# maxim2266/csvplus

Hardware: AMD Instinct MI355X
Metric: joined rows/sec (IndexOn build + chained Join, 1e8-row 3-col orders) (higher is better)
Workload: dtype u32; 1 GPU; BASELINE configs[3]: orders(1e8 x {cust_id,prod_id,qty}).Join(UniqueIndexOn customers.id 1e7).Join(UniqueIndexOn products.prod_id 1e5); rows=100000000, customers=10000000, products=100000, rows_this_rank=100000000, exchange=none (1 GPU), output=sorted positions

## Files before the change

csvplus_amd/csrc/chain.hip:

```cpp
#include <type_traits>

#include "probe_device.hpp"

namespace cph {

constexpr int kChainThreads = 256;
constexpr int kChainWaves   = kChainThreads / kWave;
constexpr int kChainRows    = 8;
constexpr int kWaveTile     = kWave * kChainRows;
constexpr int kChainTile    = kChainThreads * kChainRows;
constexpr int kChainMasks   = kChainRows * kChainWaves;
constexpr int kMaxChain     = 4;

struct ChainStepArg {
    DevCol col;
    const uint8_t* codec;
    const uint32_t* rowtab;
    const uint2* ranktab;
    int32_t positions;
    int32_t ranktab_lds;
    const uint4* hash;
    uint32_t hash_sectors;
    uint32_t hash_slice_mask;
    int32_t src;
    const uint32_t* src_perm;
    const void* codes;
    const uint32_t* perm;
    uint64_t n_index;
    int32_t codec_bytes;
    int32_t key32;
};
struct ChainArgs {
    ChainStepArg step[kMaxChain];
    uint32_t* out_rows[kMaxChain];
    int32_t nt_streams;
    int32_t reserved_;
};
struct LeanArgs {
    int32_t identity[kMaxChain];
    ArithPlan arith[kMaxChain];
};

template <int S, bool LONG, bool WIDE, bool DBG, uint32_t LEAN = 0, int R = kChainRows, bool DEP = false>
__global__ __launch_bounds__(kChainThreads) void k_chain_dense(ChainArgs a, uint64_t nprobe, uint64_t probe_base,
                                                              uint64_t ntiles, uint64_t* __restrict__ masks,
                                                              uint32_t* __restrict__ wave_counts, int dbg_flags, LeanArgs la) {
    extern __shared__ __attribute__((aligned(16))) uint8_t smem[];
    using B = std::conditional_t<WIDE, uint64_t, uint32_t>;
    using CW = std::conditional_t<WIDE, uint64_t, uint32_t>;
    const int dbg = DBG ? dbg_flags : 0;
    CodecView cv[S];
    {
        uint8_t* p = smem;
#pragma unroll
        for (int s = 0; s < S; s++) {
            if ((LEAN >> s) & 1u) continue;
            cv[s] = codec_load_to_lds(a.step[s].codec, p);
            p += a.step[s].codec_bytes;
        }
    }
    const CPH_LDS uint32_t* rank_lds[S];
    {
        uint8_t* p = smem;
#pragma unroll
        for (int s = 0; s < S; s++) p += a.step[s].codec_bytes;
        bool any = false;
#pragma unroll
        for (int s = 0; s < S; s++) {
            rank_lds[s] = nullptr;
            const int nblk = a.step[s].ranktab_lds;
            if (LEAN != 0 && nblk) {
                uint2* dst = reinterpret_cast<uint2*>(p);
                for (int i = threadIdx.x; i < 2 * nblk; i += kChainThreads) dst[i] = a.step[s].ranktab[i];
                rank_lds[s] = (const CPH_LDS uint32_t*)p;
                p += (size_t)nblk * 16;
                any = true;
            } else if (nblk) {
                uint32_t* dst = reinterpret_cast<uint32_t*>(p);
                for (int i = threadIdx.x; i < nblk; i += kChainThreads) {
                    const uint2 b0 = a.step[s].ranktab[2 * i], b1 = a.step[s].ranktab[2 * i + 1];
                    dst[3 * i] = b0.x;
                    dst[3 * i + 1] = b1.x;
                    dst[3 * i + 2] = b0.x ? b0.y : b1.y;
                }
                rank_lds[s] = (const CPH_LDS uint32_t*)p;
                p += (size_t)((nblk * 12 + 15) & ~15);
                any = true;
            }
        }
        if (any) __syncthreads();
    }
    const int lane = lane_id();
    const uint32_t wave = (uint32_t)__builtin_amdgcn_readfirstlane(wave_id());

#pragma unroll 1
    for (uint64_t tile = blockIdx.x; tile < ntiles; tile += gridDim.x) {
        uint32_t wave_matches = 0;
#pragma unroll 1
      for (int part = 0; part < kChainRows / R; part++) {
        const uint64_t wbase = tile * kChainTile + (uint64_t)wave * kWaveTile + (uint64_t)part * (R * kWave);
        const WaveRows<R> wr = wave_rows<R>(wbase, nprobe);
        uint32_t okm = wr.okm;
        WaveSpans<R, B> sp[S];
        uint64_t c0[S][R], c1[LONG ? S : 1][R];
        CW code[S][R];
        uint32_t brow[S][R];
#pragma unroll
      for (int lvl = 0; lvl < (DEP ? S : 1); lvl++) {
#pragma unroll
        for (int s = 0; s < S; s++) {
            if (DEP && s != lvl) continue;
            if ((LEAN >> s) & 1u) continue;
            if constexpr (DEP) {
                const int32_t src = a.step[s].src;
                if (src != 0) {
                    const int t = (src < 0 ? -src : src) - 1;
                    uint32_t grow[R];
#pragma unroll
                    for (int k = 0; k < R; k++) grow[k] = 0u;
#pragma unroll
                    for (int u = 0; u < S; u++)
                        if (u < s && u == t) {
#pragma unroll
                            for (int k = 0; k < R; k++) grow[k] = (okm >> k) & 1u ? brow[u][k] : 0u;
                        }
                    if (a.step[s].src_perm) {
#pragma unroll
                        for (int k = 0; k < R; k++) grow[k] = a.step[s].src_perm[grow[k]];
                    }
                    gather_spans<R, B>(a.step[s].col, grow, &sp[s]);
                    continue;
                }
            }
            if (a.nt_streams) wave_spans<R, B, false, true>(a.step[s].col, wr, &sp[s]);
            else wave_spans<R, B>(a.step[s].col, wr, &sp[s]);
        }
#pragma unroll
        for (int s = 0; s < S; s++) {
            if (DEP && s != lvl) continue;
            if ((LEAN >> s) & 1u) {
                typedef const __attribute__((address_space(1))) uint64_t* global_u64_ptr;
                const global_u64_ptr w = (global_u64_ptr)a.step[s].col.data + wr.rbase;
                if (a.nt_streams) {
#pragma unroll
                    for (int k = 0; k < R; k++) c0[s][k] = __builtin_nontemporal_load(&w[wr.rel[k]]);
                } else {
#pragma unroll
                    for (int k = 0; k < R; k++) c0[s][k] = w[wr.rel[k]];
                }
                continue;
            }
#pragma unroll
            for (int k = 0; k < R; k++) {
                c0[s][k] = a.nt_streams ? sp[s].chunk_nt(k, 0) : sp[s].chunk(k, 0);
                if constexpr (LONG) c1[s][k] = a.nt_streams ? sp[s].chunk_nt(k, 1) : sp[s].chunk(k, 1);
            }
        }
#pragma unroll
        for (int s = 0; s < S; s++) {
            if (DEP && s != lvl) continue;
            if (DBG && (dbg & 2)) {
#pragma unroll
                for (int k = 0; k < R; k++) code[s][k] = (CW)((c0[s][k] ^ (LONG ? c1[LONG ? s : 0][k] : 0ull)) & 1023);
            } else if ((LEAN >> s) & 1u) {
                encode_rows_arith<R, CW>(la.arith[s], c0[s], code[s], &okm);
            } else if (!WIDE || cv[s].hdr->lutw_bits == 32) {
                encode_rows<R, uint32_t, B, CW, LONG>(cv[s], sp[s], c0[s], c1[LONG ? s : 0], code[s], &okm,
                                                               a.step[s].col.fixed_width != 0 && (int)a.step[s].col.fixed_width == cv[s].hdr->col_maxlen[0]);
            } else {
                encode_rows<R, uint64_t, B, CW, LONG>(cv[s], sp[s], c0[s], c1[LONG ? s : 0], code[s], &okm,
                                                               a.step[s].col.fixed_width != 0 && (int)a.step[s].col.fixed_width == cv[s].hdr->col_maxlen[0]);
            }
        }
#pragma unroll
        for (int s = 0; s < S; s++) {
            if (DEP && s != lvl) continue;
            const ChainStepArg& st = a.step[s];
            if constexpr (LEAN != 0) {
                if (la.identity[s]) {
#pragma unroll
                    for (int k = 0; k < R; k++)
                        brow[s][k] = ((okm >> k) & 1u) && (uint32_t)code[s][k] < (uint32_t)st.n_index ? (uint32_t)code[s][k] : kTableAbsent;
                } else if (rank_lds[s]) {
#pragma unroll
                    for (int k = 0; k < R; k++) {
                        const uint32_t cidx = (okm >> k) & 1u ? (uint32_t)code[s][k] : 0u;
                        const CPH_LDS uint32_t* e = rank_lds[s] + 2u * (cidx >> 5);
                        const uint32_t bits = e[0], before = e[1], bit = cidx & 31u;
                        brow[s][k] = (bits >> bit) & 1u ? before + (uint32_t)__popc(bits & ((1u << bit) - 1u)) : kTableAbsent;
                    }
                } else {
                    uint2 blk[R];
#pragma unroll
                    for (int k = 0; k < R; k++) {
                        const uint32_t cidx = (okm >> k) & 1u ? (uint32_t)code[s][k] : 0u;
                        blk[k] = st.ranktab[cidx >> 5];
                    }
#pragma unroll
                    for (int k = 0; k < R; k++) {
                        const uint32_t bit = (uint32_t)code[s][k] & 31u;
                        brow[s][k] = (blk[k].x >> bit) & 1u ? blk[k].y + (uint32_t)__popc(blk[k].x & ((1u << bit) - 1u)) : kTableAbsent;
                    }
                }
            } else if (st.ranktab) {
                if (rank_lds[s]) {
#pragma unroll
                    for (int k = 0; k < R; k++) {
                        const CW cidx = (okm >> k) & 1u ? code[s][k] : (CW)0;
                        const CPH_LDS uint32_t* e = rank_lds[s] + 3u * (uint32_t)((uint64_t)cidx >> 6);
                        const uint32_t bit = (uint32_t)cidx & 63u;
                        const uint64_t bits = (uint64_t)e[0] | ((uint64_t)e[1] << 32);
                        const bool present = (bits >> bit) & 1ull;
                        brow[s][k] = present ? e[2] + (uint32_t)__popcll(bits & ((1ull << bit) - 1ull)) : kTableAbsent;
                    }
                } else {
                    uint2 blk[R];
#pragma unroll
                    for (int k = 0; k < R; k++) {
                        const CW cidx = (okm >> k) & 1u ? code[s][k] : (CW)0;
                        blk[k] = (DBG && (dbg & 1)) ? make_uint2(~0u, 0u) : st.ranktab[(uint64_t)cidx >> 5];
                    }
#pragma unroll
                    for (int k = 0; k < R; k++) {
                        const uint32_t bit = (uint32_t)code[s][k] & 31u;
                        const bool present = (blk[k].x >> bit) & 1u;
                        brow[s][k] = present ? blk[k].y + (uint32_t)__popc(blk[k].x & ((1u << bit) - 1u)) : kTableAbsent;
                    }
                }
            } else if (st.rowtab) {
#pragma unroll
                for (int k = 0; k < R; k++) {
                    const CW cidx = (okm >> k) & 1u ? code[s][k] : (CW)0;
                    brow[s][k] = (DBG && (dbg & 1)) ? 0u : st.rowtab[cidx];
                }
            } else if (st.hash) {
                const HashView hv{st.hash, st.hash_sectors, st.hash_slice_mask};
#pragma unroll
                for (int g = 0; g < R; g += 4) {
                    HashSector sc[4];
                    uint32_t home[4];
#pragma unroll
                    for (int k = 0; k < 4; k++) {
                        home[k] = hash_home(hash_one((uint64_t)code[s][g + k]), hv.nsectors);
                        sc[k] = hash_load_sector(hv, (okm >> (g + k)) & 1u ? home[k] : 0u);
                    }
#pragma unroll
                    for (int k = 0; k < 4; k++) {
                        uint32_t l, a;
                        bool more;
                        bool hit = hash_match16(sc[k], (uint64_t)code[s][g + k], &l, &a, &more);
                        const bool live = (okm >> (g + k)) & 1u;
                        if (live && more) hit = hash_continue16(hv, home[k], (uint64_t)code[s][g + k], &l, &a);
                        brow[s][g + k] = (hit && live && !(DBG && (dbg & 1))) ? (st.positions ? l : a) : kTableAbsent;
                        if (DBG && (dbg & 1)) brow[s][g + k] = 0u;
                    }
                }
            } else {
#pragma unroll
                for (int k = 0; k < R; k++) {
                    brow[s][k] = kTableAbsent;
                    if (!((okm >> k) & 1u)) continue;
                    uint64_t lo;
                    bool hit;
                    if (st.key32) {
                        const uint32_t* cd = reinterpret_cast<const uint32_t*>(st.codes);
                        lo = lower_bound_dev<uint32_t>(cd, 0, st.n_index, (uint32_t)code[s][k]);
                        hit = lo < st.n_index && cd[lo] == (uint32_t)code[s][k];
                    } else {
                        const uint64_t* cd = reinterpret_cast<const uint64_t*>(st.codes);
                        lo = lower_bound_dev<uint64_t>(cd, 0, st.n_index, (uint64_t)code[s][k]);
                        hit = lo < st.n_index && cd[lo] == (uint64_t)code[s][k];
                    }
                    if (hit) brow[s][k] = st.positions ? (uint32_t)lo : st.perm[lo];
                }
            }
        }
#pragma unroll
        for (int s = 0; s < S; s++) {
            if (DEP && s != lvl) continue;
#pragma unroll
            for (int k = 0; k < R; k++)
                if (brow[s][k] == kTableAbsent) okm &= ~(1u << k);
        }
      }
        const uint64_t mword = (tile * kChainWaves + wave) * kChainRows + (uint64_t)part * R;
#pragma unroll
        for (int k = 0; k < R; k++) {
            const bool ok = (okm >> k) & 1u;
            const uint64_t bal = __ballot(ok);
            wave_matches += (uint32_t)__popcll(bal);
            if (lane == 0) masks[mword + k] = bal;
            if (ok && !(DBG && (dbg & 4))) {
#pragma unroll
                for (int s = 0; s < S; s++) {
                    if (a.nt_streams) __builtin_nontemporal_store(brow[s][k], a.out_rows[s] + wr.rbase + wr.rel[k]);
                    else (a.out_rows[s] + wr.rbase)[wr.rel[k]] = brow[s][k];
                }
            }
        }
      }
        if (lane == 0) wave_counts[tile * kChainWaves + wave] = wave_matches;
    }
}

struct CodeStepArg {
    const uint32_t* codes;
    const uint32_t* rowtab;
    const uint2* ranktab;
    uint64_t n_index, table_entries;
    int32_t identity;
    int32_t reserved_;
};
struct CodeArgs {
    CodeStepArg step[kMaxChain];
    uint32_t* out_rows[kMaxChain];
};
template <int S>
__global__ __launch_bounds__(kChainThreads) void k_chain_codes(CodeArgs a, uint64_t nprobe, uint64_t ntiles, uint64_t* __restrict__ masks,
                                                              uint32_t* __restrict__ wave_counts) {
    const int lane = lane_id();
    const uint32_t wave = (uint32_t)__builtin_amdgcn_readfirstlane(wave_id());
#pragma unroll 1
    for (uint64_t tile = blockIdx.x; tile < ntiles; tile += gridDim.x) {
        const uint64_t wbase = tile * kChainTile + (uint64_t)wave * kWaveTile;
        const WaveRows<kChainRows> wr = wave_rows<kChainRows>(wbase, nprobe);
        uint32_t okm = wr.okm;
        uint32_t code[S][kChainRows], brow[S][kChainRows];
#pragma unroll
        for (int s = 0; s < S; s++)
#pragma unroll
            for (int k = 0; k < kChainRows; k++) code[s][k] = (a.step[s].codes + wr.rbase)[wr.rel[k]];
#pragma unroll
        for (int s = 0; s < S; s++) {
            const CodeStepArg& st = a.step[s];
            if (st.identity) {
#pragma unroll
                for (int k = 0; k < kChainRows; k++) brow[s][k] = (uint64_t)code[s][k] < st.n_index ? code[s][k] : kTableAbsent;
            } else if (st.ranktab) {
                uint2 blk[kChainRows];
#pragma unroll
                for (int k = 0; k < kChainRows; k++) {
                    const bool in = (uint64_t)code[s][k] < st.table_entries;
                    blk[k] = st.ranktab[in ? code[s][k] >> 5 : 0u];
                    if (!in) blk[k].x = 0u;
                }
#pragma unroll
                for (int k = 0; k < kChainRows; k++) {
                    const uint32_t bit = code[s][k] & 31u;
                    brow[s][k] = (blk[k].x >> bit) & 1u ? blk[k].y + (uint32_t)__popc(blk[k].x & ((1u << bit) - 1u)) : kTableAbsent;
                }
            } else {
#pragma unroll
                for (int k = 0; k < kChainRows; k++) {
                    const bool in = (uint64_t)code[s][k] < st.table_entries;
                    const uint32_t r = st.rowtab[in ? code[s][k] : 0u];
                    brow[s][k] = in ? r : kTableAbsent;
                }
            }
        }
#pragma unroll
        for (int s = 0; s < S; s++)
#pragma unroll
            for (int k = 0; k < kChainRows; k++)
                if (brow[s][k] == kTableAbsent) okm &= ~(1u << k);
        uint32_t wave_matches = 0;
        const uint64_t mword = (tile * kChainWaves + wave) * kChainRows;
#pragma unroll
        for (int k = 0; k < kChainRows; k++) {
            const bool ok = (okm >> k) & 1u;
            const uint64_t bal = __ballot(ok);
            wave_matches += (uint32_t)__popcll(bal);
            if (lane == 0) masks[mword + k] = bal;
            if (ok) {
#pragma unroll
                for (int s = 0; s < S; s++) (a.out_rows[s] + wr.rbase)[wr.rel[k]] = brow[s][k];
            }
        }
        if (lane == 0) wave_counts[tile * kChainWaves + wave] = wave_matches;
    }
}

__global__ __launch_bounds__(256) void k_sum_counts(const uint32_t* __restrict__ counts, uint64_t n,
                                                   unsigned long long* __restrict__ total) {
    __shared__ uint64_t s_w[256 / kWave];
    uint64_t t = 0;
    const uint64_t stride = (uint64_t)gridDim.x * 256;
    for (uint64_t i = (uint64_t)blockIdx.x * 256 + threadIdx.x; i < n; i += stride) t += counts[i];
    t = wave_sum(t);
    if (lane_id() == 0) s_w[wave_id()] = t;
    __syncthreads();
    if (threadIdx.x == 0) {
        uint64_t r = 0;
        for (int w = 0; w < 256 / kWave; w++) r += s_w[w];
        if (r) atomicAdd(total, (unsigned long long)r);
    }
}

__global__ __launch_bounds__(256) void k_sum_counts_report(const uint32_t* __restrict__ counts, uint64_t n, unsigned long long* __restrict__ acc,
                                                          uint32_t* __restrict__ ticket, unsigned long long* __restrict__ host_out) {
    __shared__ uint64_t s_w[256 / kWave];
    uint64_t t = 0;
    const uint64_t stride = (uint64_t)gridDim.x * 256;
    for (uint64_t i = (uint64_t)blockIdx.x * 256 + threadIdx.x; i < n; i += stride) t += counts[i];
    t = wave_sum(t);
    if (lane_id() == 0) s_w[wave_id()] = t;
    __syncthreads();
    if (threadIdx.x == 0) {
        uint64_t r = 0;
        for (int w = 0; w < 256 / kWave; w++) r += s_w[w];
        if (r) atomicAdd(acc, (unsigned long long)r);
        __threadfence();
        if (atomicAdd(ticket, 1u) == gridDim.x - 1u) {
            const unsigned long long total = atomicExch(acc, 0ull);
            atomicExch(ticket, 0u);
            *host_out = total;
            __threadfence_system();
        }
    }
}

template <int S>
__global__ __launch_bounds__(kChainThreads) void k_chain_compact(ChainArgs dense_rows, uint64_t probe_base,
                                                                const uint64_t* __restrict__ masks,
                                                                const uint32_t* __restrict__ wave_base, uint64_t ntiles,
                                                                uint64_t* __restrict__ out_stream, ChainArgs out_rows) {
    const int lane = lane_id(), wave = wave_id();
    const uint64_t lt = lanemask_lt();
    for (uint64_t tile = blockIdx.x; tile < ntiles; tile += gridDim.x) {
        const uint64_t wt = tile * kChainWaves + wave;
        uint64_t pos = wave_base[wt];
#pragma unroll
        for (int k = 0; k < kChainRows; k++) {
            const uint64_t m = masks[wt * kChainRows + k];
            if ((m >> lane) & 1ull) {
                const uint64_t row = wt * kWaveTile + (uint64_t)k * kWave + lane;
                const uint64_t p = pos + (uint64_t)__popcll(m & lt);
                out_stream[p] = probe_base + row;
#pragma unroll
                for (int s = 0; s < S; s++) out_rows.out_rows[s][p] = dense_rows.out_rows[s][row];
            }
            pos += (uint64_t)__popcll(m);
        }
    }
}

__global__ void k_compose_u64(const uint64_t* __restrict__ src, const uint64_t* __restrict__ idx, uint64_t* __restrict__ dst,
                              uint64_t n) {
    const uint64_t stride = (uint64_t)gridDim.x * blockDim.x;
    for (uint64_t i = (uint64_t)blockIdx.x * blockDim.x + threadIdx.x; i < n; i += stride) dst[i] = src[idx[i]];
}
__global__ void k_compose_u32(const uint32_t* __restrict__ src, const uint64_t* __restrict__ idx, uint32_t* __restrict__ dst,
                              uint64_t n) {
    const uint64_t stride = (uint64_t)gridDim.x * blockDim.x;
    for (uint64_t i = (uint64_t)blockIdx.x * blockDim.x + threadIdx.x; i < n; i += stride) dst[i] = src[idx[i]];
}

__global__ void k_perm_rows(const uint32_t* __restrict__ perm, const uint32_t* __restrict__ pos, uint32_t* __restrict__ dst, uint64_t n) {
    const uint64_t stride = (uint64_t)gridDim.x * blockDim.x;
    for (uint64_t i = (uint64_t)blockIdx.x * blockDim.x + threadIdx.x; i < n; i += stride) dst[i] = perm[pos[i]];
}

__global__ void k_gather_rows(const uint32_t* __restrict__ tab, const uint32_t* __restrict__ idx, uint32_t* __restrict__ dst, uint64_t n) {
    const uint64_t stride = (uint64_t)gridDim.x * blockDim.x;
    for (uint64_t i = (uint64_t)blockIdx.x * blockDim.x + threadIdx.x; i < n; i += stride) dst[i] = tab[idx[i]];
}

struct PrejoinArgs {
    int32_t n;
    int32_t src_dep[kMaxChain - 1];
    const uint32_t* src_rows[kMaxChain - 1];
    const uint32_t* tab[kMaxChain - 1];
    uint32_t* out_rows[kMaxChain - 1];
};
__global__ __launch_bounds__(kChainThreads) void k_chain_prejoined(PrejoinArgs a, uint64_t nprobe, uint64_t ntiles, uint64_t* __restrict__ masks,
                                                                  uint32_t* __restrict__ wave_counts) {
    const int lane = lane_id();
    const uint32_t wave = (uint32_t)__builtin_amdgcn_readfirstlane(wave_id());
#pragma unroll 1
    for (uint64_t tile = blockIdx.x; tile < ntiles; tile += gridDim.x) {
        const uint64_t wbase = tile * kChainTile + (uint64_t)wave * kWaveTile;
        const uint64_t mword = (tile * kChainWaves + wave) * kChainRows;
        uint32_t okm = 0;
#pragma unroll
        for (int k = 0; k < kChainRows; k++) okm |= (uint32_t)((masks[mword + k] >> lane) & 1ull) << k;
        uint32_t val[kMaxChain - 1][kChainRows];
#pragma unroll
        for (int j = 0; j < kMaxChain - 1; j++) {
            if (j >= a.n) break;
            uint32_t h[kChainRows];
            const int sd = a.src_dep[j];
            if (sd < 0) {
#pragma unroll
                for (int k = 0; k < kChainRows; k++) {
                    const uint64_t r = wbase + (uint64_t)k * kWave + lane;
                    h[k] = (okm >> k) & 1u ? a.src_rows[j][r] : 0u;
                }
            } else {
#pragma unroll
                for (int k = 0; k < kChainRows; k++) h[k] = 0u;
#pragma unroll
                for (int u = 0; u < kMaxChain - 1; u++)
                    if (u < j && u == sd) {
#pragma unroll
                        for (int k = 0; k < kChainRows; k++) h[k] = (okm >> k) & 1u ? val[u][k] : 0u;
                    }
            }
#pragma unroll
            for (int k = 0; k < kChainRows; k++) val[j][k] = a.tab[j][h[k]];
#pragma unroll
            for (int k = 0; k < kChainRows; k++)
                if (val[j][k] == kTableAbsent) okm &= ~(1u << k);
        }
        uint32_t wave_matches = 0;
#pragma unroll
        for (int k = 0; k < kChainRows; k++) {
            const bool ok = (okm >> k) & 1u;
            const uint64_t bal = __ballot(ok);
            wave_matches += (uint32_t)__popcll(bal);
            if (lane == 0) masks[mword + k] = bal;
            if (ok) {
                const uint64_t r = wbase + (uint64_t)k * kWave + lane;
#pragma unroll
                for (int j = 0; j < kMaxChain - 1; j++)
                    if (j < a.n) __builtin_nontemporal_store(val[j][k], a.out_rows[j] + r);
            }
        }
        if (lane == 0) wave_counts[tile * kChainWaves + wave] = wave_matches;
    }
}


constexpr int kPjThreads = 256, kPjItems = 8, kPjTile = kPjThreads * kPjItems;
__global__ __launch_bounds__(kPjThreads) void k_prejoin_tuples(const uint32_t* __restrict__ tab, const uint32_t* __restrict__ h,
                                                              const uint32_t* __restrict__ perm, uint64_t n,
                                                              uint32_t* __restrict__ out_v, uint32_t* __restrict__ tile_counts) {
    __shared__ uint32_t s_w[kPjThreads / kWave];
    const uint64_t base = (uint64_t)blockIdx.x * kPjTile;
    uint32_t hv[kPjItems], v[kPjItems];
#pragma unroll
    for (int k = 0; k < kPjItems; k++) {
        const uint64_t i = base + (uint64_t)k * kPjThreads + threadIdx.x;
        hv[k] = i < n ? __builtin_nontemporal_load(h + i) : 0u;
    }
    if (perm) {
#pragma unroll
        for (int k = 0; k < kPjItems; k++) hv[k] = perm[hv[k]];
    }
#pragma unroll
    for (int k = 0; k < kPjItems; k++) v[k] = tab[hv[k]];
    uint32_t cnt = 0;
#pragma unroll
    for (int k = 0; k < kPjItems; k++) {
        const uint64_t i = base + (uint64_t)k * kPjThreads + threadIdx.x;
        if (i < n) {
            __builtin_nontemporal_store(v[k], out_v + i);
            cnt += v[k] != kTableAbsent ? 1u : 0u;
        }
    }
    cnt = wave_sum(cnt);
    if (lane_id() == 0) s_w[wave_id()] = cnt;
    __syncthreads();
    if (threadIdx.x == 0) {
        uint32_t t = 0;
        for (int w = 0; w < kPjThreads / kWave; w++) t += s_w[w];
        tile_counts[blockIdx.x] = t;
    }
}
struct PjCompactArgs {
    int32_t n32;
    const uint32_t* src32[CPH_MAX_CHAIN];
    uint32_t* dst32[CPH_MAX_CHAIN];
    const uint64_t* src64;
    uint64_t* dst64;
};
__global__ __launch_bounds__(kPjThreads) void k_prejoin_compact(PjCompactArgs a, const uint32_t* __restrict__ v, uint64_t n,
                                                               const uint32_t* __restrict__ tile_base) {
    __shared__ uint32_t s_tmp[kPjThreads / kWave + 1];
    const uint64_t i0 = (uint64_t)blockIdx.x * kPjTile + (uint64_t)threadIdx.x * kPjItems;
    uint32_t keep = 0, mine = 0;
#pragma unroll
    for (int k = 0; k < kPjItems; k++)
        if (i0 + k < n && v[i0 + k] != kTableAbsent) {
            keep |= 1u << k;
            mine++;
        }
    uint32_t total;
    uint32_t run = block_exclusive_sum<uint32_t, kPjThreads>(mine, s_tmp, &total);
    uint64_t o = (uint64_t)tile_base[blockIdx.x] + run;
#pragma unroll
    for (int k = 0; k < kPjItems; k++) {
        if (!((keep >> k) & 1u)) continue;
        a.dst64[o] = a.src64[i0 + k];
        for (int j = 0; j < a.n32; j++) a.dst32[j][o] = a.src32[j][i0 + k];
        o++;
    }
}

bool chain_fast_path_ok(const ChainStep* steps, int nsteps) {
    if (nsteps > kMaxChain) return false;
    for (int s = 0; s < nsteps; s++) {
        const cph_index* ix = steps[s].index;
        if (steps[s].ncols != 1 || ix->nkeycols != 1) return false;
        if (ix->first_dup != UINT64_MAX) return false;
        if (ix->codec.nwords != 1 || ix->codec.npos == 0 || !ix->windows.empty()) return false;
// ... 526 lines not shown
```

csvplus_amd/csrc/codec_device.hpp:

```cpp
#pragma once

#include "cph_internal.hpp"
#include "device_utils.hpp"

namespace cph {

__device__ __forceinline__ uint64_t find_first_byte(const uint8_t* data, uint64_t begin, uint64_t len, uint32_t d) {
    const uint64_t dv = 0x0101010101010101ull * (uint64_t)(d & 0xFFu);
    for (uint64_t j = 0; 8 * j < len; j++) {
        const uint64_t x = load_value_chunk(data, begin, len, (int)j) ^ dv;
        const uint64_t t = (x - 0x0101010101010101ull) & ~x & 0x8080808080808080ull;
        if (t) {
            const uint64_t pos = 8 * j + (uint64_t)((__ffsll((long long)t) - 1) >> 3);
            return pos < len ? pos : len;
        }
    }
    return len;
}

__device__ __forceinline__ void value_span_whole(const DevCol& col, uint64_t row, uint64_t* begin, uint64_t* len);
__device__ __forceinline__ void value_span(const DevCol& col, uint64_t row, uint64_t* begin, uint64_t* len) {
    value_span_whole(col, row, begin, len);
    if (col.split) {
        const uint64_t b = *begin, l = *len;
        const uint64_t at = find_first_byte(col.data, b, l, col.split);
        const uint64_t head = at < l ? at + 1 : l;
        if (col.part == 0) {
            *len = head;
        } else {
            *begin = b + head;
            *len = l - head;
        }
    }
}
__device__ __forceinline__ void value_span_whole(const DevCol& col, uint64_t row, uint64_t* begin, uint64_t* len) {
    uint64_t b, l;
    if (col.fixed_width) {
        b = row * (uint64_t)col.fixed_width;
        l = col.fixed_width;
    } else {
        b = load_offset(col.offsets, col.offset_bits, row);
        l = load_offset(col.offsets, col.offset_bits, row + 1) - b;
    }
    const uint64_t s = l < (uint64_t)col.skip ? l : (uint64_t)col.skip;
    b += s;
    l -= s;
    if (col.take != 0xFFFFFFFFu && l > (uint64_t)col.take) l = col.take;
    *begin = b;
    *len = l;
}

#define CPH_LDS __attribute__((address_space(3)))

struct CodecView {
    const CPH_LDS CodecDevHeader* hdr;
    const CPH_LDS uint64_t* mult;
    const CPH_LDS uint8_t* word_of;
    const CPH_LDS uint16_t* lut;
    const CPH_LDS uint8_t* lutw;
    const CPH_LDS uint8_t* unit;
    const CPH_LDS int32_t* dict_off;
    const CPH_LDS int32_t* dict_len;
    const CPH_LDS uint64_t* dict;
    const CPH_LDS int32_t* hash_off;
    const CPH_LDS int32_t* hash_bits;
    const CPH_LDS uint16_t* hash;
    const CPH_LDS WideKey* wide;
    const CPH_LDS uint16_t* wide_hash;
    const CPH_LDS uint16_t* wide_disp;
};

__device__ __forceinline__ CodecView codec_load_to_lds(const uint8_t* g_blob, uint8_t* lds) {
    const CodecDevHeader* gh = reinterpret_cast<const CodecDevHeader*>(g_blob);
    const int total = gh->total_bytes;
    const uint4* src = reinterpret_cast<const uint4*>(g_blob);
    uint4* dst = reinterpret_cast<uint4*>(lds);
    for (int i = threadIdx.x; i < total / 16; i += blockDim.x) dst[i] = src[i];
    __syncthreads();
    const CPH_LDS uint8_t* l = (const CPH_LDS uint8_t*)lds;
    CodecView v;
    v.hdr = (const CPH_LDS CodecDevHeader*)l;
    v.mult = (const CPH_LDS uint64_t*)(l + v.hdr->mult_off);
    v.word_of = l + v.hdr->wordof_off;
    v.lut = (const CPH_LDS uint16_t*)(l + v.hdr->lut_off);
    v.lutw = l + v.hdr->lutw_off;
    v.unit = l + v.hdr->unit_off;
    v.dict_off = (const CPH_LDS int32_t*)(l + v.hdr->dictoff_off);
    v.dict_len = (const CPH_LDS int32_t*)(l + v.hdr->dictlen_off);
    v.dict = (const CPH_LDS uint64_t*)(l + v.hdr->dict_off);
    v.hash_off = (const CPH_LDS int32_t*)(l + v.hdr->hashoff_off);
    v.hash_bits = (const CPH_LDS int32_t*)(l + v.hdr->hashbits_off);
    v.hash = (const CPH_LDS uint16_t*)(l + v.hdr->hash_off);
    v.wide = (const CPH_LDS WideKey*)(l + v.hdr->wide_off);
    v.wide_hash = (const CPH_LDS uint16_t*)(l + v.hdr->wide_hash_off);
    v.wide_disp = (const CPH_LDS uint16_t*)(l + v.hdr->wide_disp_off);
    return v;
}

__device__ __forceinline__ uint32_t wide_slot(const CodecView& cv, uint32_t h) {
    const uint32_t disp = cv.wide_disp[h & ((1u << cv.hdr->wide_disp_bits) - 1u)];
    return ((h >> 16) + disp) & ((1u << cv.hdr->wide_hash_bits) - 1u);
}
__device__ __forceinline__ int wide_lookup(const CodecView& cv, uint64_t w0, uint64_t w1, uint64_t w2, uint64_t w3, uint32_t len) {
    const uint32_t e = cv.wide_hash[wide_slot(cv, wide_hash_lo(w0, w1, w2, w3, len))];
    if (e == 0) return -1;
    const CPH_LDS WideKey* k = cv.wide + (e - 1);
    return k->len == len && k->w[0] == w0 && k->w[1] == w1 && k->w[2] == w2 && k->w[3] == w3 ? (int)(e - 1) : -1;
}
__device__ __forceinline__ void wide_words(const uint8_t* data, uint64_t begin, uint64_t len, uint64_t (&w)[4]) {
#pragma unroll
    for (int j = 0; j < 4; j++) {
        uint64_t v = 0;
        if (8ull * (uint64_t)j < len) {
            v = load_value_chunk(data, begin, len, j);
            const uint64_t nb = len - 8ull * (uint64_t)j;
            if (nb < 8) v &= (1ull << (8 * nb)) - 1ull;
        }
        w[j] = v;
    }
}

template <class W>
__device__ __forceinline__ bool encode_key_premultiplied(const CodecView& cv, const ColsArg& cols, int ncols_used,
                                                         uint64_t row, uint64_t* code) {
    const CPH_LDS W* lutw = (const CPH_LDS W*)cv.lutw;
    W acc = 0, bad = 0;
    bool valid = true;
    for (int c = 0; c < ncols_used; c++) {
        const DevCol& col = cols.c[c];
        uint64_t begin, len;
        value_span(col, row, &begin, &len);
        const int maxlen = cv.hdr->col_maxlen[c];
        const CPH_LDS W* lp = lutw + cv.hdr->col_start[c] * kLutStride;
        if (len > (uint64_t)maxlen) valid = false;
        uint64_t chunk = 0;
        for (int q = 0; q < maxlen; q++) {
            if ((q & 7) == 0 && (uint64_t)q < len) chunk = load_value_chunk(col.data, begin, len, q >> 3);
            const int sym = (uint64_t)q < len ? (int)((chunk >> (8 * (q & 7))) & 0xFF) + 1 : 0;
            const W v = lp[q * kLutStride + sym];
            bad |= v;
            acc += v;
        }
    }
    *code = (uint64_t)acc;
    return valid && !(bad >> (sizeof(W) * 8 - 1));
}

template <class W>
__device__ __forceinline__ bool encode_prefetched_w(const CodecView& cv, const DevCol& col, uint64_t begin, uint32_t len,
                                                    uint64_t c0, uint64_t c1, uint64_t* code) {
    const int maxlen = cv.hdr->col_maxlen[0];
    const CPH_LDS W* lutw = (const CPH_LDS W*)cv.lutw;
    W acc = 0, bad = 0;
    uint64_t chunk = c0;
    for (int q = 0; q < maxlen; q++) {
        if ((q & 7) == 0) {
            if (q == 8) chunk = c1;
            else if (q >= 16 && (uint32_t)q < len) chunk = load_value_chunk(col.data, begin, len, q >> 3);
        }
        const uint32_t sym = (uint32_t)q < len ? ((uint32_t)(chunk >> (8 * (q & 7))) & 0xFFu) + 1u : 0u;
        const W v = lutw[q * kLutStride + sym];
        bad |= v;
        acc += v;
    }
    *code = (uint64_t)acc;
    return len <= (uint32_t)maxlen && !(bad >> (sizeof(W) * 8 - 1));
}

template <int R>
struct WaveRows {
    uint64_t rbase;
    uint32_t nvalid;
    uint32_t rel[R];
    uint32_t okm;
};
template <int R>
__device__ __forceinline__ WaveRows<R> wave_rows(uint64_t wbase, uint64_t nrows ) {
    WaveRows<R> w;
    const uint64_t left = nrows > wbase ? nrows - wbase : 0;
    w.nvalid = left > (uint64_t)(R * kWave) ? (uint32_t)(R * kWave) : (uint32_t)left;
    w.rbase = w.nvalid ? wbase : nrows - 1;
    const uint32_t rmax = w.nvalid ? w.nvalid - 1 : 0;
    w.okm = 0;
    const uint32_t lane = (uint32_t)lane_id();
#pragma unroll
    for (int k = 0; k < R; k++) {
        const uint32_t r = (uint32_t)k * kWave + lane;
        w.okm |= (r < w.nvalid ? 1u : 0u) << k;
        w.rel[k] = r < rmax ? r : rmax;
    }
    return w;
}

template <int R, class B>
struct WaveSpans {
    const uint8_t* base8;
    uint32_t delta;
    B x[R];
    uint32_t len[R];
    __device__ __forceinline__ uint64_t chunk(int k, uint32_t j) const {
        return load_chunk_nobranch<B>(base8, delta, x[k], len[k], j);
    }
    __device__ __forceinline__ uint64_t chunk_nt(int k, uint32_t j) const {
        return load_chunk_nobranch<B, true>(base8, delta, x[k], len[k], j);
    }
};
template <int R, class B, bool SEG = false, bool NT = false>
__device__ __forceinline__ void wave_spans(const DevCol& c, const WaveRows<R>& wr, WaveSpans<R, B>* sp);
template <int R, class B, bool NT = false>
__device__ __forceinline__ void wave_spans_whole(const DevCol& c, const WaveRows<R>& wr, WaveSpans<R, B>* sp);
template <int R, class B, bool SEG, bool NT>
__device__ __forceinline__ void wave_spans(const DevCol& c, const WaveRows<R>& wr, WaveSpans<R, B>* sp) {
    wave_spans_whole<R, B, NT>(c, wr, sp);
    if constexpr (SEG) {
#pragma unroll
        for (int k = 0; k < R; k++) {
            const uint32_t s = sp->len[k] < c.skip ? sp->len[k] : c.skip;
            sp->x[k] += (B)s;
            uint32_t l = sp->len[k] - s;
            if (c.take != 0xFFFFFFFFu && l > c.take) l = c.take;
            sp->len[k] = l;
        }
    }
}
template <int R, class B, bool NT>
__device__ __forceinline__ void wave_spans_whole(const DevCol& c, const WaveRows<R>& wr, WaveSpans<R, B>* sp) {
    if (c.fixed_width) {
        const uint64_t p = (uint64_t)(uintptr_t)c.data + wr.rbase * (uint64_t)c.fixed_width;
        sp->base8 = (const uint8_t*)(uintptr_t)(p & ~7ull);
        sp->delta = (uint32_t)(p & 7ull);
#pragma unroll
        for (int k = 0; k < R; k++) {
            sp->x[k] = (B)wr.rel[k] * c.fixed_width;
            sp->len[k] = c.fixed_width;
        }
        return;
    }
    const uint64_t p = (uint64_t)(uintptr_t)c.data;
    sp->base8 = (const uint8_t*)(uintptr_t)(p & ~7ull);
    sp->delta = (uint32_t)(p & 7ull);
    if (c.offset_bits == 32) {
        const uint32_t* off = reinterpret_cast<const uint32_t*>(c.offsets) + wr.rbase;
        uint32_t b[R], e[R];
#pragma unroll
        for (int k = 0; k < R; k++) {
            b[k] = NT ? __builtin_nontemporal_load(&off[wr.rel[k]]) : off[wr.rel[k]];
            e[k] = NT ? __builtin_nontemporal_load(&off[wr.rel[k] + 1]) : off[wr.rel[k] + 1];
        }
#pragma unroll
        for (int k = 0; k < R; k++) {
            sp->x[k] = b[k];
            sp->len[k] = e[k] - b[k];
        }
    } else if constexpr (sizeof(B) == 8) {
        const uint64_t* off = reinterpret_cast<const uint64_t*>(c.offsets) + wr.rbase;
        uint64_t b[R], e[R];
#pragma unroll
        for (int k = 0; k < R; k++) {
            b[k] = off[wr.rel[k]];
            e[k] = off[wr.rel[k] + 1];
        }
#pragma unroll
        for (int k = 0; k < R; k++) {
            sp->x[k] = b[k];
            const uint64_t l = e[k] - b[k];
            sp->len[k] = l > 0xFFFFFFFFull ? 0xFFFFFFFFu : (uint32_t)l;
        }
    } else {
#pragma unroll
        for (int k = 0; k < R; k++) { sp->x[k] = 0; sp->len[k] = 0; }
    }
}
template <int R, class B>
__device__ __forceinline__ void gather_spans(const DevCol& c, const uint32_t (&row)[R], WaveSpans<R, B>* sp) {
    const uint64_t p = (uint64_t)(uintptr_t)c.data;
    sp->base8 = (const uint8_t*)(uintptr_t)(p & ~7ull);
    sp->delta = (uint32_t)(p & 7ull);
    if (c.fixed_width) {
#pragma unroll
        for (int k = 0; k < R; k++) {
            sp->x[k] = (B)row[k] * (B)c.fixed_width;
            sp->len[k] = c.fixed_width;
        }
        return;
    }
    if (c.offset_bits == 32) {
        const uint32_t* off = reinterpret_cast<const uint32_t*>(c.offsets);
        uint32_t b[R], e[R];
#pragma unroll
        for (int k = 0; k < R; k++) {
            b[k] = off[row[k]];
            e[k] = off[(uint64_t)row[k] + 1];
        }
#pragma unroll
        for (int k = 0; k < R; k++) {
            sp->x[k] = b[k];
            sp->len[k] = e[k] - b[k];
        }
    } else if constexpr (sizeof(B) == 8) {
        const uint64_t* off = reinterpret_cast<const uint64_t*>(c.offsets);
        uint64_t b[R], e[R];
#pragma unroll
        for (int k = 0; k < R; k++) {
            b[k] = off[row[k]];
            e[k] = off[(uint64_t)row[k] + 1];
        }
#pragma unroll
        for (int k = 0; k < R; k++) {
            sp->x[k] = b[k];
            const uint64_t l = e[k] - b[k];
            sp->len[k] = l > 0xFFFFFFFFull ? 0xFFFFFFFFu : (uint32_t)l;
        }
    } else {
#pragma unroll
        for (int k = 0; k < R; k++) { sp->x[k] = 0; sp->len[k] = 0; }
    }
}
inline bool col_is_narrow(const DevCol& c) { return c.fixed_width ? c.fixed_width <= 0xFFFFu : c.offset_bits == 32; }

template <int R, class W, class B, bool FIXED>
__device__ __forceinline__ void encode_position(const CPH_LDS W* lp, int b, uint32_t pos, const WaveSpans<R, B>& sp, const uint64_t (&cur)[R],
                                                W (&acc)[R], W (&bad)[R]) {
#pragma unroll
    for (int k = 0; k < R; k++) {
        const uint32_t half = b < 4 ? (uint32_t)cur[k] : (uint32_t)(cur[k] >> 32);
        const uint32_t byte = (half >> (8 * (b & 3))) & 0xFFu;
        const uint32_t sym = FIXED ? byte + 1u : (pos < sp.len[k] ? byte + 1u : 0u);
        const W v = lp[b * kLutStride + sym];
        if constexpr (sizeof(W) == 4) {
            acc[k] = __builtin_elementwise_add_sat(acc[k], v);
        } else {
            bad[k] |= v;
            acc[k] += v;
        }
    }
}

template <int R, class W, class B, class CW, bool LONG>
__device__ __forceinline__ void encode_rows(const CodecView& cv, const WaveSpans<R, B>& sp, const uint64_t (&c0)[R],
                                            const uint64_t (&c1)[R], CW (&code)[R], uint32_t* okmask, bool fixed = false) {
    const int maxlen = cv.hdr->col_maxlen[0];
    const CPH_LDS W* lutw = (const CPH_LDS W*)cv.lutw;
    W acc[R], bad[R];
#pragma unroll
    for (int k = 0; k < R; k++) { acc[k] = 0; bad[k] = 0; }
    const int nchunks = (maxlen + 7) >> 3;
#pragma unroll 1
    for (int j = 0; j < nchunks; j++) {
        uint64_t cur[R];
        if (j == 0) {
#pragma unroll
            for (int k = 0; k < R; k++) cur[k] = c0[k];
        } else if (LONG && j == 1) {
#pragma unroll
            for (int k = 0; k < R; k++) cur[k] = c1[k];
        } else {
#pragma unroll
            for (int k = 0; k < R; k++) cur[k] = sp.chunk(k, (uint32_t)j);
        }
        const int qn = maxlen - 8 * j < 8 ? maxlen - 8 * j : 8;
        const CPH_LDS W* lp = lutw + (8 * j) * kLutStride;
        if (fixed) {
#pragma unroll
            for (int b = 0; b < 8; b++)
                if (b < qn) encode_position<R, W, B, true>(lp, b, (uint32_t)(8 * j + b), sp, cur, acc, bad);
        } else {
#pragma unroll
            for (int b = 0; b < 8; b++)
                if (b < qn) encode_position<R, W, B, false>(lp, b, (uint32_t)(8 * j + b), sp, cur, acc, bad);
        }
    }
    uint32_t m = *okmask;
#pragma unroll
    for (int k = 0; k < R; k++) {
        code[k] = (CW)acc[k];
        const W flag = sizeof(W) == 4 ? acc[k] : bad[k];
        const bool good = sp.len[k] <= (uint32_t)maxlen && !(flag >> (sizeof(W) * 8 - 1));
        if (!good) m &= ~(1u << k);
    }
    *okmask = m;
}

struct ArithPlan {
    uint32_t enabled;
    uint32_t mul24;
    uint32_t keylen;
    uint32_t keep[2];
    uint32_t lo[2];
    uint32_t rngc[2];
    uint32_t wa[2], wb[2];
    uint32_t ma[2];
    uint32_t s1;
};

void codec_arith_plan(const CodecHost& codec, ArithPlan* ap);

template <int R, class CW>
__device__ __forceinline__ void encode_rows_arith(const ArithPlan& ap, const uint64_t (&c0)[R], CW (&code)[R], uint32_t* okmask) {
    uint32_t m = *okmask;
    uint32_t zl[R], zh[R];
#pragma unroll
    for (int k = 0; k < R; k++) {
        const uint32_t xl = (uint32_t)c0[k], xh = (uint32_t)(c0[k] >> 32);
        zl[k] = xl - ap.lo[0];
        zh[k] = xh - ap.lo[1];
        const uint32_t tl = zl[k] + ap.rngc[0], th = zh[k] + ap.rngc[1];
        const uint32_t bad = ((xl | zl[k] | tl) | (xh | zh[k] | th)) & 0x80808080u;
        if (bad) m &= ~(1u << k);
    }
    if (ap.mul24) {
#pragma unroll
        for (int k = 0; k < R; k++) {
            const uint32_t pa0 = __builtin_amdgcn_udot4(zl[k], ap.wa[0], 0u, false);
            const uint32_t pa1 = __builtin_amdgcn_udot4(zh[k], ap.wa[1], 0u, false);
            const uint32_t w0 = __builtin_amdgcn_udot4(zl[k], ap.wb[0], __umul24(pa0, ap.ma[0]), false);
            code[k] = (CW)__builtin_amdgcn_udot4(zh[k], ap.wb[1], __umul24(pa1, ap.ma[1]) + __umul24(w0, ap.s1), false);
        }
    } else {
#pragma unroll
        for (int k = 0; k < R; k++) {
            const uint32_t pa0 = __builtin_amdgcn_udot4(zl[k], ap.wa[0], 0u, false);
            const uint32_t pa1 = __builtin_amdgcn_udot4(zh[k], ap.wa[1], 0u, false);
            const uint32_t w0 = __builtin_amdgcn_udot4(zl[k], ap.wb[0], pa0 * ap.ma[0], false);
            code[k] = (CW)__builtin_amdgcn_udot4(zh[k], ap.wb[1], pa1 * ap.ma[1] + w0 * ap.s1, false);
        }
    }
    *okmask = m;
}

template <bool LONGV = true>
struct ValueHeadT {
    uint64_t begin = 0, len = 0, c0 = 0, c1 = 0, c2 = 0;
    __device__ __forceinline__ void span(const DevCol& col, uint64_t row) { value_span(col, row, &begin, &len); }
    __device__ __forceinline__ void chunks(const DevCol& col) {
        c0 = len > 0 ? load_value_chunk(col.data, begin, len, 0) : 0;
        c1 = len > 8 ? load_value_chunk(col.data, begin, len, 1) : 0;
        c2 = len > 16 ? load_value_chunk(col.data, begin, len, 2) : 0;
    }
    __device__ __forceinline__ void chunks_nobranch(const DevCol& col) {
        const uint64_t p = (uint64_t)(uintptr_t)col.data;
        const uint8_t* base8 = (const uint8_t*)(uintptr_t)(p & ~7ull);
        const uint32_t delta = (uint32_t)(p & 7ull);
        const uint32_t l32 = len > 0xFFFFFFFFull ? 0xFFFFFFFFu : (uint32_t)len;
        const uint64_t a = load_chunk_nobranch<uint64_t>(base8, delta, begin, l32, 0);
        const uint64_t b = load_chunk_nobranch<uint64_t>(base8, delta, begin, l32, 1);
        const uint64_t c = load_chunk_nobranch<uint64_t>(base8, delta, begin, l32, 2);
        c0 = l32 > 0 ? a : 0;
        c1 = l32 > 8 ? b : 0;
        c2 = l32 > 16 ? c : 0;
    }
    __device__ __forceinline__ void load(const DevCol& col, uint64_t row) {
        span(col, row);
        chunks(col);
    }
    __device__ __forceinline__ uint64_t chunk(const DevCol& col, int j) const {
        if constexpr (LONGV) {
            if (8ull * (uint64_t)j >= len) return 0;
            return j == 0 ? c0 : j == 1 ? c1 : j == 2 ? c2 : load_value_chunk(col.data, begin, len, j);
        } else {
            return j == 0 ? c0 : j == 1 ? c1 : j == 2 ? c2 : 0;
        }
    }
    __device__ __forceinline__ uint32_t sym(const DevCol& col, int q) const {
        const uint32_t b = ((uint32_t)(chunk(col, q >> 3) >> (8 * (q & 7))) & 0xFFu) + 1u;
        return (uint64_t)q < len ? b : 0u;
    }
    __device__ __forceinline__ uint64_t window(const DevCol& col, int q) const {
        const int sh = (q & 7) * 8;
        const uint64_t lo = chunk(col, q >> 3);
        if (sh == 0) return lo;
        return (lo >> sh) | (chunk(col, (q >> 3) + 1) << (64 - sh));
    }
    __device__ __forceinline__ uint64_t raw(const DevCol& col, int q, int span) const {
        const uint64_t nvalid = len > (uint64_t)q ? (len - (uint64_t)q < (uint64_t)span ? len - (uint64_t)q : (uint64_t)span) : 0;
        return group_raw(window(col, q), nvalid);
    }
    template <int J>
    __device__ __forceinline__ uint64_t ck() const {
        if constexpr (J == 0) return c0;
        else if constexpr (J == 1) return c1;
        else if constexpr (J == 2) return c2;
        else return 0;
    }
    template <int J>
    __device__ __forceinline__ uint32_t sym_j(int q) const {
        const uint32_t b = ((uint32_t)(ck<J>() >> (8 * (q & 7))) & 0xFFu) + 1u;
        return (uint64_t)q < len ? b : 0u;
    }
    template <int J>
    __device__ __forceinline__ uint64_t window_j(int q) const {
        const int sh = (q & 7) * 8;
        return sh == 0 ? ck<J>() : (ck<J>() >> sh) | (ck<J + 1>() << (64 - sh));
    }
    template <int J>
    __device__ __forceinline__ uint64_t raw_j(int q, int span) const {
        const uint32_t l32 = len > 0xFFFFFFFFull ? 0xFFFFFFFFu : (uint32_t)len;
        const uint32_t left = l32 > (uint32_t)q ? l32 - (uint32_t)q : 0u;
        return group_raw(window_j<J>(q), (uint64_t)(left < (uint32_t)span ? left : (uint32_t)span));
    }
};
using ValueHead = ValueHeadT<true>;

template <class Emit>
__device__ __forceinline__ bool encode_key_groups(const CodecView& cv, const ColsArg& cols, int ncols_used, uint64_t row,
                                                  Emit&& emit) {
    const int p_end = cv.hdr->col_start[ncols_used];
    uint64_t acc = 0;
    bool valid = true;
    for (int c = 0; c < ncols_used; c++) {
        const DevCol& col = cols.c[c];
        uint64_t begin, len;
        value_span(col, row, &begin, &len);
        const int maxlen = cv.hdr->col_maxlen[c];
        const int p0 = cv.hdr->col_start[c];
        if (len > (uint64_t)maxlen) valid = false;
        ValueHead v;
        v.begin = begin;
        v.len = len;
        v.chunks(col);
        for (int q = 0; q < maxlen; q++) {
            const int p = p0 + q;
            const uint32_t kind = cv.unit[p];
            uint64_t r = 0;
            if (kind == kUnitWide) {
                int rank = -1;
                if (len <= (uint64_t)kWideBytes) {
                    uint64_t w[4];
                    wide_words(col.data, begin, len, w);
                    rank = wide_lookup(cv, w[0], w[1], w[2], w[3], (uint32_t)len);
                }
                if (rank < 0) valid = false;
                r = rank < 0 ? 0ull : (uint64_t)rank;
            } else if (kind == kUnitHead) {
                int span = 1;
                while (span < kGroupSpan && q + span < maxlen && cv.unit[p + span] == kUnitAbsorbed) span++;
                const uint64_t joint = v.raw(col, q, span);
                const CPH_LDS uint64_t* d = cv.dict + cv.dict_off[p];
                const CPH_LDS uint16_t* ht = cv.hash + cv.hash_off[p];
                const int bits = cv.hash_bits[p];
                const uint32_t mask = (1u << bits) - 1u;
                uint32_t sl = bits ? group_slot(joint, bits) : 0u;
                bool found = false;
                for (;;) {
                    const uint32_t e = ht[sl];
                    if (e == 0) break;
                    if (d[e - 1] == joint) { r = (uint64_t)(e - 1); found = true; break; }
                    sl = (sl + 1) & mask;
                }
                if (!found) valid = false;
            } else if (kind == kUnitPos) {
                const uint32_t rr = cv.lut[p * kLutStride + (int)v.sym(col, q)];
                if (rr == kLutInvalid) valid = false;
                r = rr;
            }
            acc += r * cv.mult[p];
            if (p + 1 == p_end || cv.word_of[p + 1] != cv.word_of[p]) {
                emit((int)cv.word_of[p], acc, p);
                acc = 0;
            }
        }
    }
    return valid;
}

template <class Emit>
__device__ __forceinline__ bool encode_key(const CodecView& cv, const ColsArg& cols, int ncols_used, uint64_t row,
                                           Emit&& emit) {
    const int p_end = cv.hdr->col_start[ncols_used];
    if (cv.hdr->lutw_bits != 0) {
        uint64_t code;
        const bool valid = cv.hdr->lutw_bits == 32 ? encode_key_premultiplied<uint32_t>(cv, cols, ncols_used, row, &code)
                                                   : encode_key_premultiplied<uint64_t>(cv, cols, ncols_used, row, &code);
        if (p_end > 0) emit(0, code, p_end - 1);
        return valid;
    }
    if (cv.hdr->ngroups != 0) return encode_key_groups(cv, cols, ncols_used, row, emit);
    uint64_t acc = 0;
    bool valid = true;
    for (int c = 0; c < ncols_used; c++) {
        const DevCol& col = cols.c[c];
        uint64_t begin, len;
        value_span(col, row, &begin, &len);
        const int maxlen = cv.hdr->col_maxlen[c];
        const int p0 = cv.hdr->col_start[c];
        if (len > (uint64_t)maxlen) valid = false;
        uint64_t chunk = 0;
        for (int q = 0; q < maxlen; q++) {
            if ((q & 7) == 0 && (uint64_t)q < len) chunk = load_value_chunk(col.data, begin, len, q >> 3);
            const int sym = (uint64_t)q < len ? (int)((chunk >> (8 * (q & 7))) & 0xFF) + 1 : 0;
            const int p = p0 + q;
            const uint32_t r = cv.lut[p * kLutStride + sym];
            if (r == kLutInvalid) valid = false;
            acc += (uint64_t)r * cv.mult[p];
            if (p + 1 == p_end || cv.word_of[p + 1] != cv.word_of[p]) {
                emit((int)cv.word_of[p], acc, p);
                acc = 0;
            }
        }
    }
    return valid;
}

}
```

Before: 133.4 billion rows/s.

## Add specialized lean chain tile path with full-tile fast path and boolean masks

Result: no change. 132.8 billion rows/s (-0.4%).

```diff
diff --git a/csvplus_amd/csrc/chain.hip b/csvplus_amd/csrc/chain.hip
--- a/csvplus_amd/csrc/chain.hip
+++ b/csvplus_amd/csrc/chain.hip
@@ -41,6 +41,118 @@
     ArithPlan arith[kMaxChain];
 };
 
+template <int S, uint32_t LEAN, bool FULL>
+__device__ __forceinline__ uint32_t chain_lean_tile(const ChainArgs& a, const LeanArgs& la, const CodecView (&cv)[S],
+                                                    const CPH_LDS uint32_t* const (&rank_lds)[S], uint64_t wbase, uint64_t nprobe,
+                                                    uint64_t* __restrict__ mwords) {
+    constexpr int R = kChainRows;
+    typedef uint32_t u32x2 __attribute__((ext_vector_type(2)));
+    typedef const __attribute__((address_space(1))) uint64_t* global_u64_ptr;
+    typedef const __attribute__((address_space(1))) u32x2* global_u32x2_ptr;
+    const WaveRows<R> wr = FULL ? wave_rows_full<R>(wbase) : wave_rows<R>(wbase, nprobe);
+    WaveSpans<R, uint32_t> sp[S];
+    uint64_t c0[S][R];
+    uint32_t code[S][R], brow[S][R];
+    bool good[S][R], hit[S][R];
+#pragma unroll
+    for (int s = 0; s < S; s++) {
+        if ((LEAN >> s) & 1u) continue;
+        if (a.nt_streams) wave_spans<R, uint32_t, false, true>(a.step[s].col, wr, &sp[s]);
+        else wave_spans<R, uint32_t>(a.step[s].col, wr, &sp[s]);
+    }
+#pragma unroll
+    for (int s = 0; s < S; s++) {
+        if ((LEAN >> s) & 1u) {
+            const global_u64_ptr w = (global_u64_ptr)a.step[s].col.data + wr.rbase;
+            if (a.nt_streams) {
+#pragma unroll
+                for (int k = 0; k < R; k++) c0[s][k] = __builtin_nontemporal_load(&w[wr.rel[k]]);
+            } else {
+#pragma unroll
+                for (int k = 0; k < R; k++) c0[s][k] = w[wr.rel[k]];
+            }
+        } else if (a.nt_streams) {
+#pragma unroll
+            for (int k = 0; k < R; k++) c0[s][k] = sp[s].chunk_nt(k, 0);
+        } else {
+#pragma unroll
+            for (int k = 0; k < R; k++) c0[s][k] = sp[s].chunk(k, 0);
+        }
+    }
+#pragma unroll
+    for (int s = 0; s < S; s++) {
+        if ((LEAN >> s) & 1u)
+            encode_rows_arith<R, uint32_t>(la.arith[s], c0[s], code[s], good[s]);
+        else
+            encode_rows<R, uint32_t, uint32_t, uint32_t, false>(cv[s], sp[s], c0[s], c0[s], code[s], good[s],
+                                                                a.step[s].col.fixed_width != 0 && (int)a.step[s].col.fixed_width == cv[s].hdr->col_maxlen[0]);
+    }
+#pragma unroll
+    for (int s = 0; s < S; s++) {
+        const ChainStepArg& st = a.step[s];
+        if (la.identity[s]) {
+#pragma unroll
+            for (int k = 0; k < R; k++) {
+                hit[s][k] = good[s][k] && code[s][k] < (uint32_t)st.n_index;
+                brow[s][k] = code[s][k];
+            }
+            continue;
+        }
+        u32x2 blk[R];
+        if (rank_lds[s]) {
+            const CPH_LDS u32x2* rt = (const CPH_LDS u32x2*)rank_lds[s];
+#pragma unroll
+            for (int k = 0; k < R; k++) blk[k] = rt[(good[s][k] ? code[s][k] : 0u) >> 5];
+        } else {
+            const global_u32x2_ptr rt = (global_u32x2_ptr)st.ranktab;
+#pragma unroll
+            for (int k = 0; k < R; k++) blk[k] = rt[(good[s][k] ? code[s][k] : 0u) >> 5];
+        }
+#pragma unroll
+        for (int k = 0; k < R; k++) {
+            const uint32_t bit = code[s][k] & 31u;
+            hit[s][k] = good[s][k] && ((blk[k].x >> bit) & 1u);
+            brow[s][k] = blk[k].y + (uint32_t)__popc(blk[k].x & ((1u << bit) - 1u));
+        }
+    }
+    bool ok[R];
+    uint64_t bal[R], all = ~0ull;
+    uint32_t matches = 0;
+#pragma unroll
+    for (int k = 0; k < R; k++) {
+        ok[k] = FULL || ((wr.okm >> k) & 1u);
+#pragma unroll
+        for (int s = 0; s < S; s++) ok[k] = ok[k] && hit[s][k];
+        bal[k] = __ballot(ok[k]);
+        matches += (uint32_t)__popcll(bal[k]);
+        all &= bal[k];
+    }
+    if (lane_id() == 0) {
+#pragma unroll
+        for (int k = 0; k < R; k++) mwords[k] = bal[k];
+    }
+    auto store_rows = [&](auto every, auto nt) {
+#pragma unroll
+        for (int k = 0; k < R; k++) {
+            if (!decltype(every)::value && !ok[k]) continue;
+#pragma unroll
+            for (int s = 0; s < S; s++) {
+                uint32_t* dst = a.out_rows[s] + wr.rbase + wr.rel[k];
+                if constexpr (decltype(nt)::value) __builtin_nontemporal_store(brow[s][k], dst);
+                else *dst = brow[s][k];
+            }
+        }
+    };
+    if (all == ~0ull) {
+        if (a.nt_streams) store_rows(std::true_type{}, std::true_type{});
+        else store_rows(std::true_type{}, std::false_type{});
+    } else {
+        if (a.nt_streams) store_rows(std::false_type{}, std::true_type{});
+        else store_rows(std::false_type{}, std::false_type{});
+    }
+    return matches;
+}
+
 template <int S, bool LONG, bool WIDE, bool DBG, uint32_t LEAN = 0, int R = kChainRows, bool DEP = false>
 __global__ __launch_bounds__(kChainThreads) void k_chain_dense(ChainArgs a, uint64_t nprobe, uint64_t probe_base,
                                                               uint64_t ntiles, uint64_t* __restrict__ masks,
@@ -93,6 +205,17 @@
     const int lane = lane_id();
     const uint32_t wave = (uint32_t)__builtin_amdgcn_readfirstlane(wave_id());
 
+    if constexpr (LEAN != 0) {
+#pragma unroll 1
+        for (uint64_t tile = blockIdx.x; tile < ntiles; tile += gridDim.x) {
+            const uint64_t wt = tile * kChainWaves + wave;
+            const uint64_t wbase = wt * kWaveTile;
+            uint32_t wave_matches;
+            if (wbase + kWaveTile <= nprobe) wave_matches = chain_lean_tile<S, LEAN, true>(a, la, cv, rank_lds, wbase, nprobe, masks + wt * kChainRows);
+            else wave_matches = chain_lean_tile<S, LEAN, false>(a, la, cv, rank_lds, wbase, nprobe, masks + wt * kChainRows);
+            if (lane == 0) wave_counts[wt] = wave_matches;
+        }
+    } else {
 #pragma unroll 1
     for (uint64_t tile = blockIdx.x; tile < ntiles; tile += gridDim.x) {
         uint32_t wave_matches = 0;
@@ -110,7 +233,6 @@
 #pragma unroll
         for (int s = 0; s < S; s++) {
             if (DEP && s != lvl) continue;
-            if ((LEAN >> s) & 1u) continue;
             if constexpr (DEP) {
                 const int32_t src = a.step[s].src;
                 if (src != 0) {
@@ -138,18 +260,6 @@
 #pragma unroll
         for (int s = 0; s < S; s++) {
             if (DEP && s != lvl) continue;
-            if ((LEAN >> s) & 1u) {
-                typedef const __attribute__((address_space(1))) uint64_t* global_u64_ptr;
-                const global_u64_ptr w = (global_u64_ptr)a.step[s].col.data + wr.rbase;
-                if (a.nt_streams) {
-#pragma unroll
-                    for (int k = 0; k < R; k++) c0[s][k] = __builtin_nontemporal_load(&w[wr.rel[k]]);
-                } else {
-#pragma unroll
-                    for (int k = 0; k < R; k++) c0[s][k] = w[wr.rel[k]];
-                }
-                continue;
-            }
 #pragma unroll
             for (int k = 0; k < R; k++) {
                 c0[s][k] = a.nt_streams ? sp[s].chunk_nt(k, 0) : sp[s].chunk(k, 0);
@@ -162,8 +272,6 @@
             if (DBG && (dbg & 2)) {
 #pragma unroll
                 for (int k = 0; k < R; k++) code[s][k] = (CW)((c0[s][k] ^ (LONG ? c1[LONG ? s : 0][k] : 0ull)) & 1023);
-            } else if ((LEAN >> s) & 1u) {
-                encode_rows_arith<R, CW>(la.arith[s], c0[s], code[s], &okm);
             } else if (!WIDE || cv[s].hdr->lutw_bits == 32) {
                 encode_rows<R, uint32_t, B, CW, LONG>(cv[s], sp[s], c0[s], c1[LONG ? s : 0], code[s], &okm,
                                                                a.step[s].col.fixed_width != 0 && (int)a.step[s].col.fixed_width == cv[s].hdr->col_maxlen[0]);
@@ -176,33 +284,7 @@
         for (int s = 0; s < S; s++) {
             if (DEP && s != lvl) continue;
             const ChainStepArg& st = a.step[s];
-            if constexpr (LEAN != 0) {
-                if (la.identity[s]) {
-#pragma unroll
-                    for (int k = 0; k < R; k++)
-                        brow[s][k] = ((okm >> k) & 1u) && (uint32_t)code[s][k] < (uint32_t)st.n_index ? (uint32_t)code[s][k] : kTableAbsent;
-                } else if (rank_lds[s]) {
-#pragma unroll
-                    for (int k = 0; k < R; k++) {
-                        const uint32_t cidx = (okm >> k) & 1u ? (uint32_t)code[s][k] : 0u;
-                        const CPH_LDS uint32_t* e = rank_lds[s] + 2u * (cidx >> 5);
-                        const uint32_t bits = e[0], before = e[1], bit = cidx & 31u;
-                        brow[s][k] = (bits >> bit) & 1u ? before + (uint32_t)__popc(bits & ((1u << bit) - 1u)) : kTableAbsent;
-                    }
-                } else {
-                    uint2 blk[R];
-#pragma unroll
-                    for (int k = 0; k < R; k++) {
-                        const uint32_t cidx = (okm >> k) & 1u ? (uint32_t)code[s][k] : 0u;
-                        blk[k] = st.ranktab[cidx >> 5];
-                    }
-#pragma unroll
-                    for (int k = 0; k < R; k++) {
-                        const uint32_t bit = (uint32_t)code[s][k] & 31u;
-                        brow[s][k] = (blk[k].x >> bit) & 1u ? blk[k].y + (uint32_t)__popc(blk[k].x & ((1u << bit) - 1u)) : kTableAbsent;
-                    }
-                }
-            } else if (st.ranktab) {
+            if (st.ranktab) {
                 if (rank_lds[s]) {
 #pragma unroll
                     for (int k = 0; k < R; k++) {
@@ -300,6 +382,7 @@
         }
       }
         if (lane == 0) wave_counts[tile * kChainWaves + wave] = wave_matches;
+    }
     }
 }
 
diff --git a/csvplus_amd/csrc/codec_device.hpp b/csvplus_amd/csrc/codec_device.hpp
--- a/csvplus_amd/csrc/codec_device.hpp
+++ b/csvplus_amd/csrc/codec_device.hpp
@@ -192,6 +192,18 @@
     return w;
 }
 
+template <int R>
+__device__ __forceinline__ WaveRows<R> wave_rows_full(uint64_t wbase) {
+    WaveRows<R> w;
+    w.rbase = wbase;
+    w.nvalid = (uint32_t)(R * kWave);
+    w.okm = (1u << R) - 1u;
+    const uint32_t lane = (uint32_t)lane_id();
+#pragma unroll
+    for (int k = 0; k < R; k++) w.rel[k] = (uint32_t)k * kWave + lane;
+    return w;
+}
+
 template <int R, class B>
 struct WaveSpans {
     const uint8_t* base8;
@@ -338,7 +350,7 @@
 
 template <int R, class W, class B, class CW, bool LONG>
 __device__ __forceinline__ void encode_rows(const CodecView& cv, const WaveSpans<R, B>& sp, const uint64_t (&c0)[R],
-                                            const uint64_t (&c1)[R], CW (&code)[R], uint32_t* okmask, bool fixed = false) {
+                                            const uint64_t (&c1)[R], CW (&code)[R], bool (&good)[R], bool fixed = false) {
     const int maxlen = cv.hdr->col_maxlen[0];
     const CPH_LDS W* lutw = (const CPH_LDS W*)cv.lutw;
     W acc[R], bad[R];
@@ -370,14 +382,22 @@
                 if (b < qn) encode_position<R, W, B, false>(lp, b, (uint32_t)(8 * j + b), sp, cur, acc, bad);
         }
     }
-    uint32_t m = *okmask;
 #pragma unroll
     for (int k = 0; k < R; k++) {
         code[k] = (CW)acc[k];
         const W flag = sizeof(W) == 4 ? acc[k] : bad[k];
-        const bool good = sp.len[k] <= (uint32_t)maxlen && !(flag >> (sizeof(W) * 8 - 1));
-        if (!good) m &= ~(1u << k);
-    }
+        good[k] = sp.len[k] <= (uint32_t)maxlen && !(flag >> (sizeof(W) * 8 - 1));
+    }
+}
+template <int R, class W, class B, class CW, bool LONG>
+__device__ __forceinline__ void encode_rows(const CodecView& cv, const WaveSpans<R, B>& sp, const uint64_t (&c0)[R],
+                                            const uint64_t (&c1)[R], CW (&code)[R], uint32_t* okmask, bool fixed = false) {
+    bool good[R];
+    encode_rows<R, W, B, CW, LONG>(cv, sp, c0, c1, code, good, fixed);
+    uint32_t m = *okmask;
+#pragma unroll
+    for (int k = 0; k < R; k++)
+        if (!good[k]) m &= ~(1u << k);
     *okmask = m;
 }
 
@@ -396,8 +416,7 @@
 void codec_arith_plan(const CodecHost& codec, ArithPlan* ap);
 
 template <int R, class CW>
-__device__ __forceinline__ void encode_rows_arith(const ArithPlan& ap, const uint64_t (&c0)[R], CW (&code)[R], uint32_t* okmask) {
-    uint32_t m = *okmask;
+__device__ __forceinline__ void encode_rows_arith(const ArithPlan& ap, const uint64_t (&c0)[R], CW (&code)[R], bool (&good)[R]) {
     uint32_t zl[R], zh[R];
 #pragma unroll
     for (int k = 0; k < R; k++) {
@@ -405,8 +424,7 @@
         zl[k] = xl - ap.lo[0];
         zh[k] = xh - ap.lo[1];
         const uint32_t tl = zl[k] + ap.rngc[0], th = zh[k] + ap.rngc[1];
-        const uint32_t bad = ((xl | zl[k] | tl) | (xh | zh[k] | th)) & 0x80808080u;
-        if (bad) m &= ~(1u << k);
+        good[k] = (((xl | zl[k] | tl) | (xh | zh[k] | th)) & 0x80808080u) == 0u;
     }
     if (ap.mul24) {
 #pragma unroll
@@ -425,6 +443,15 @@
             code[k] = (CW)__builtin_amdgcn_udot4(zh[k], ap.wb[1], pa1 * ap.ma[1] + w0 * ap.s1, false);
         }
     }
+}
+template <int R, class CW>
+__device__ __forceinline__ void encode_rows_arith(const ArithPlan& ap, const uint64_t (&c0)[R], CW (&code)[R], uint32_t* okmask) {
+    bool good[R];
+    encode_rows_arith<R, CW>(ap, c0, code, good);
+    uint32_t m = *okmask;
+#pragma unroll
+    for (int k = 0; k < R; k++)
+        if (!good[k]) m &= ~(1u << k);
     *okmask = m;
 }
 
```
